# microsoft/XPretrain

Hardware: NVIDIA H100
Metric: video-text pairs/sec (12f x 224^2, 32 tok), CLIP-ViP ViT-B/16 fwd+InfoNCE+bwd (higher is better)
Workload: dtype bf16

## Files before the change

### xpretrain_b200/csrc/gemm.cu

```cuda
#include "../../include/xpretrain_b200.h"
#include "common.h"
#include "ptx.cuh"
#include <cstdlib>

namespace xp {

constexpr int BM = 128;
constexpr int BK = 64;
constexpr int MMA_K = 16;
constexpr int GEMM_THREADS = 384;

struct GemmDev {
  void* c;
  const float* bias;
  const __nv_bfloat16* residual;
  __nv_bfloat16* aux;
  int M, N, K;
  long long ldc, ldr, ld_aux;
  long long c_group, c_group_stride, r_group, r_group_stride;
  int act;
  int splits;
  int scale_cols;
  float alpha, col_scale;
  uint32_t mn_lbo, mn_sbo;
};

template <int BN>
struct GemmCfg {
  static constexpr int A_BYTES = BM * BK * 2;
  static constexpr int B_BYTES = BN * BK * 2;
  static constexpr int STAGE_BYTES = A_BYTES + B_BYTES;
  static constexpr int STAGES = (BN == 256) ? 4 : 6;
  static constexpr int SMEM_BYTES = STAGES * STAGE_BYTES + 1024 + 256;
};

__device__ __forceinline__ float act_gelu_erf(float x) { return 0.5f * x * (1.f + erff(x * 0.70710678118654752f)); }
__device__ __forceinline__ float act_gelu_erf_grad(float x) {
  float cdf = 0.5f * (1.f + erff(x * 0.70710678118654752f));
  float pdf = 0.3989422804014327f * __expf(-0.5f * x * x);
  return cdf + x * pdf;
}

template <int BN, int A_MN, int B_MN, int OUT, int ACT>
__global__ void __launch_bounds__(GEMM_THREADS, 1)
gemm_kernel(const __grid_constant__ CUtensorMap tmA, const __grid_constant__ CUtensorMap tmB, const GemmDev p) {
  using Cfg = GemmCfg<BN>;
  constexpr int STAGES = Cfg::STAGES;
  constexpr bool PINGPONG = BN == 128;
  constexpr int MH = PINGPONG ? 2 : 1;
  constexpr int NH = BN / 128;
  extern __shared__ uint8_t smem_raw[];
  const uint32_t raw_addr = smem_u32(smem_raw);
  uint8_t* smem = smem_raw + (((raw_addr + 1023u) & ~1023u) - raw_addr);
  uint64_t* full_bar = reinterpret_cast<uint64_t*>(smem + STAGES * Cfg::STAGE_BYTES);
  uint64_t* empty_bar = full_bar + STAGES;

  const int wg = threadIdx.x >> 7;
  const int lane = threadIdx.x & 31;

  const int num_m = (p.M + BM - 1) / BM;
  const int num_n = (p.N + BN - 1) / BN;
  const int num_mn = num_m * num_n;
  const int total = num_mn * p.splits;
  const int kb_total = (p.K + BK - 1) / BK;
  const int kb_per = (kb_total + p.splits - 1) / p.splits;

  if (threadIdx.x == 0) {
    tma_prefetch_desc(&tmA);
    tma_prefetch_desc(&tmB);
    for (int s = 0; s < STAGES; ++s) {
      mbar_init(&full_bar[s], 1);
      mbar_init(&empty_bar[s], PINGPONG ? 1 : 2);
    }
    fence_barrier_init();
  }
  __syncthreads();

  if (wg == 0) {
    setmaxnreg_dec<40>();
    if (threadIdx.x == 0) {
      int stage = 0;
      uint32_t phase = 0;
      for (int tile = blockIdx.x; tile < total; tile += gridDim.x) {
        const int split = tile / num_mn;
        const int mn = tile - split * num_mn;
        const int m_blk = mn / num_n;
        const int n_blk = mn - m_blk * num_n;
        const int k0 = split * kb_per;
        const int k1 = min(kb_total, k0 + kb_per);
        for (int kb = k0; kb < k1; ++kb) {
          mbar_wait_nocall(&empty_bar[stage], phase ^ 1);
          uint8_t* sA = smem + stage * Cfg::STAGE_BYTES;
          uint8_t* sB = sA + Cfg::A_BYTES;
          mbar_arrive_expect_tx(&full_bar[stage], Cfg::STAGE_BYTES);
          if (A_MN) {
#pragma unroll
            for (int i = 0; i < BM / 64; ++i)
              tma_load_2d(sA + i * (BK * 128), &tmA, &full_bar[stage], m_blk * BM + i * 64, kb * BK);
          } else {
            tma_load_2d(sA, &tmA, &full_bar[stage], kb * BK, m_blk * BM);
          }
          if (B_MN) {
#pragma unroll
            for (int i = 0; i < BN / 64; ++i)
              tma_load_2d(sB + i * (BK * 128), &tmB, &full_bar[stage], n_blk * BN + i * 64, kb * BK);
          } else {
            tma_load_2d(sB, &tmB, &full_bar[stage], kb * BK, n_blk * BN);
          }
          if (++stage == STAGES) {
            stage = 0;
            phase ^= 1;
          }
        }
      }
    }
  } else {
    setmaxnreg_inc<232>();
    const int cw = wg - 1;
    const int wq = (threadIdx.x >> 5) & 3;
    constexpr int act = ACT;
    const int N = p.N, scale_cols = p.scale_cols;
    const float alpha = p.alpha, col_scale = p.col_scale;
    __nv_bfloat16* const aux_p = p.aux;
    constexpr bool need_aux_in = (ACT == XP_ACT_DQUICK_GELU || ACT == XP_ACT_DGELU_ERF);
    const __nv_bfloat16* const xin_p = need_aux_in ? p.aux : p.residual;
    constexpr uint32_t A_OFF = 64 * 128;
    const int cta_tiles = (total - blockIdx.x + gridDim.x - 1) / gridDim.x;
    int stage = 0;
    uint32_t phase = 0;
    int local = 0;
    for (int tile = blockIdx.x; tile < total; tile += gridDim.x, ++local) {
      const int split = tile / num_mn;
      const int mn = tile - split * num_mn;
      const int m_blk = mn / num_n;
      const int n_blk = mn - m_blk * num_n;
      const int k0 = split * kb_per;
      const int k1 = min(kb_total, k0 + kb_per);
      if (PINGPONG && (local & 1) != cw) {
        const int next = stage + max(0, k1 - k0);
        phase ^= (next / STAGES) & 1;
        stage = next % STAGES;
        continue;
      }
      if (PINGPONG && local > 0) named_bar_sync(1 + cw, 256);
      const bool pass_turn = PINGPONG && local + 1 < cta_tiles;
      if (k0 >= k1) {
        if (pass_turn) named_bar_arrive(2 - cw, 256);
        continue;
      }
      float acc[MH * NH][64];
#pragma unroll
      for (int q = 0; q < MH * NH; ++q)
#pragma unroll
        for (int i = 0; i < 64; ++i) acc[q][i] = 0.f;
      int prev_stage = -1;
      for (int kb = k0; kb < k1; ++kb) {
        mbar_wait_nocall(&full_bar[stage], phase);
        const uint32_t sA = smem_u32(smem + stage * Cfg::STAGE_BYTES) + (PINGPONG ? 0 : cw * A_OFF);
        const uint32_t sB = smem_u32(smem + stage * Cfg::STAGE_BYTES) + Cfg::A_BYTES;
#pragma unroll
        for (int q = 0; q < MH * NH; ++q) wgmma_fence_regs(acc[q]);
        wgmma_fence();
#pragma unroll
        for (int j = 0; j < BK / MMA_K; ++j) {
#pragma unroll
          for (int mh = 0; mh < MH; ++mh) {
            const uint32_t am = sA + mh * A_OFF;
            const uint64_t adesc = A_MN ? make_smem_desc_sw128(am + j * (MMA_K * 128), p.mn_lbo, p.mn_sbo)
                                        : make_smem_desc_sw128(am + j * (MMA_K * 2), 16, 1024);
#pragma unroll
            for (int h = 0; h < NH; ++h) {
              const uint32_t bh = sB + h * (128 * 128);
              const uint64_t bdesc = B_MN ? make_smem_desc_sw128(bh + j * (MMA_K * 128), p.mn_lbo, p.mn_sbo)
                                          : make_smem_desc_sw128(bh + j * (MMA_K * 2), 16, 1024);
              wgmma_m64n128k16_bf16<A_MN, B_MN>(acc[mh * NH + h], adesc, bdesc);
            }
          }
        }
        wgmma_commit();
#pragma unroll
        for (int q = 0; q < MH * NH; ++q) wgmma_fence_regs(acc[q]);
        wgmma_wait<1>();
        if (prev_stage >= 0 && (threadIdx.x & 127) == 0) mbar_arrive(&empty_bar[prev_stage]);
        prev_stage = stage;
        if (++stage == STAGES) {
          stage = 0;
          phase ^= 1;
        }
      }
      if (pass_turn) named_bar_arrive(2 - cw, 256);
      const auto load_bias = [&](float2(&b)[16], int h) {
#pragma unroll
        for (int i = 0; i < 16; ++i) {
          const int n = n_blk * BN + h * 128 + i * 8 + (lane & 3) * 2;
          b[i] = make_float2(0.f, 0.f);
          if (p.bias != nullptr && split == 0 && n < N) b[i] = __ldg(reinterpret_cast<const float2*>(p.bias + n));
        }
      };
      constexpr bool bias_once = PINGPONG && !need_aux_in;
      float2 bias_tile[16];
      if (bias_once) load_bias(bias_tile, 0);
      wgmma_wait<0>();
#pragma unroll
      for (int q = 0; q < MH * NH; ++q) wgmma_fence_regs(acc[q]);
      if ((threadIdx.x & 127) == 0) mbar_arrive(&empty_bar[prev_stage]);

      const auto apply = [&](float& v0, float& v1, int n, uint32_t xg) -> uint32_t {
        if (n < scale_cols) {
          v0 *= col_scale;
          v1 *= col_scale;
        }
        uint32_t pre = 0;
        if (act == XP_ACT_QUICK_GELU) {
          pre = pack_bf16(v0, v1);
          v0 = quick_gelu(v0);
          v1 = quick_gelu(v1);
        } else if (act == XP_ACT_DQUICK_GELU) {
          v0 *= quick_gelu_grad(bf16_lo(xg));
          v1 *= quick_gelu_grad(bf16_hi(xg));
        } else if (act == XP_ACT_GELU_ERF) {
          pre = pack_bf16(v0, v1);
          v0 = act_gelu_erf(v0);
          v1 = act_gelu_erf(v1);
        } else if (act == XP_ACT_DGELU_ERF) {
          v0 *= act_gelu_erf_grad(bf16_lo(xg));
          v1 *= act_gelu_erf_grad(bf16_hi(xg));
        } else if (xin_p != nullptr) {
          v0 += bf16_lo(xg);
          v1 += bf16_hi(xg);
        }
        return pre;
      };
      constexpr bool save_pre = (ACT == XP_ACT_QUICK_GELU || ACT == XP_ACT_GELU_ERF);
      const int quad = lane & 3;
#pragma unroll
      for (int mh = 0; mh < MH; ++mh) {
        const int row_base = m_blk * BM + (PINGPONG ? mh : cw) * 64 + wq * 16 + (lane >> 2);
#pragma unroll
        for (int rr = 0; rr < 2; ++rr) {
          const int row = row_base + rr * 8;
          const bool row_ok = row < p.M;
          const long long c_off = p.c_group > 0 ? (row / p.c_group) * p.c_group_stride + (row % p.c_group) * p.ldc
                                                : static_cast<long long>(row) * p.ldc;
          const long long x_off = need_aux_in ? static_cast<long long>(row) * p.ld_aux
                                              : (p.r_group > 0 ? (row / p.r_group) * p.r_group_stride + (row % p.r_group) * p.ldr
                                                               : static_cast<long long>(row) * p.ldr);
          const long long a_off = static_cast<long long>(row) * p.ld_aux;
#pragma unroll
          for (int h = 0; h < NH; ++h) {
            const float* const a = acc[mh * NH + h];
            const int n_h = n_blk * BN + h * 128;
            float2 bias2[16];
            if (bias_once) {
#pragma unroll
              for (int i = 0; i < 16; ++i) bias2[i] = bias_tile[i];
            } else {
              load_bias(bias2, h);
            }
            if (OUT == XP_OUT_BF16) {
              uint32_t xin[4][4];
#pragma unroll
              for (int k = 0; k < 4; ++k) {
                const int n8 = n_h + (4 * k + quad) * 8;
                uint4 v = make_uint4(0u, 0u, 0u, 0u);
                if (xin_p != nullptr && row_ok && n8 < N) v = *reinterpret_cast<const uint4*>(xin_p + x_off + n8);
                xin[k][0] = v.x;
                xin[k][1] = v.y;
                xin[k][2] = v.z;
                xin[k][3] = v.w;
                if (xin_p != nullptr) quad_transpose(xin[k]);
              }
#pragma unroll
              for (int k = 0; k < 4; ++k) {
                uint32_t out[4], pre[4];
#pragma unroll
                for (int j = 0; j < 4; ++j) {
                  const int i = 4 * k + j;
                  float v0 = fmaf(a[4 * i + 2 * rr], alpha, bias2[i].x);
                  float v1 = fmaf(a[4 * i + 2 * rr + 1], alpha, bias2[i].y);
                  pre[j] = apply(v0, v1, n_h + i * 8 + quad * 2, xin[k][j]);
                  out[j] = pack_bf16(v0, v1);
                }
                const int n8 = n_h + (4 * k + quad) * 8;
                quad_transpose(out);
                if (row_ok && n8 < N)
                  *reinterpret_cast<uint4*>(static_cast<__nv_bfloat16*>(p.c) + c_off + n8) =
                      make_uint4(out[0], out[1], out[2], out[3]);
                if (save_pre && aux_p != nullptr) {
                  quad_transpose(pre);
                  if (row_ok && n8 < N)
                    *reinterpret_cast<uint4*>(aux_p + a_off + n8) = make_uint4(pre[0], pre[1], pre[2], pre[3]);
                }
              }
            } else if (row_ok) {
              uint32_t xin[16];
#pragma unroll
              for (int i = 0; i < 16; ++i) {
                const int n = n_h + i * 8 + quad * 2;
                xin[i] = 0;
                if (xin_p != nullptr && n < N) xin[i] = *reinterpret_cast<const uint32_t*>(xin_p + x_off + n);
              }
#pragma unroll
              for (int i = 0; i < 16; ++i) {
                const int n = n_h + i * 8 + quad * 2;
                if (n >= N) continue;
                float v0 = fmaf(a[4 * i + 2 * rr], alpha, bias2[i].x);
                float v1 = fmaf(a[4 * i + 2 * rr + 1], alpha, bias2[i].y);
                apply(v0, v1, n, xin[i]);
                if (OUT == XP_OUT_F32) {
                  *reinterpret_cast<float2*>(static_cast<float*>(p.c) + c_off + n) = make_float2(v0, v1);
                } else {
                  asm volatile("red.global.add.v2.f32 [%0], {%1, %2};" ::"l"(static_cast<float*>(p.c) + c_off + n),
                               "f"(v0), "f"(v1)
                               : "memory");
                }
              }
            }
          }
        }
      }
    }
  }
}

static int g_dbg_mn_lbo = 0, g_dbg_mn_sbo = 0;
}

extern "C" void xp_debug_gemm_mn_desc(int lbo, int sbo) {
  xp::g_dbg_mn_lbo = lbo;
  xp::g_dbg_mn_sbo = sbo;
}

extern "C" int xp_gemm(const XpGemm* g, void* stream_v) {
  using namespace xp;
  if (!g) return fail("xp_gemm: null args");
  cudaStream_t stream = static_cast<cudaStream_t>(stream_v);
  if (g->M <= 0 || g->N <= 0 || g->K <= 0) return fail("xp_gemm: M, N, K must be positive");
  if (g->N % 8 != 0) return fail("xp_gemm: N must be a multiple of 8");
  if (!g->a || !g->b || !g->c) return fail("xp_gemm: null operand");
  XP_ENTER(g->a);
  const int splits = g->splits <= 0 ? 1 : g->splits;
  if (splits > 1 && g->out != XP_OUT_F32_ATOMIC) return fail("xp_gemm: split-K requires XP_OUT_F32_ATOMIC");
  if ((g->act == XP_ACT_DQUICK_GELU || g->act == XP_ACT_DGELU_ERF) && !g->aux)
    return fail("xp_gemm: dGELU epilogue needs aux (the forward pre-activation)");
  if (g->act != XP_ACT_NONE && g->out != XP_OUT_BF16) return fail("xp_gemm: activation epilogues need a bf16 output");
  if (g->act != XP_ACT_NONE && g->residual)
    return fail("xp_gemm: a residual add cannot be combined with an activation epilogue");
  if (g->aux && g->c_group > 0) return fail("xp_gemm: aux cannot be combined with grouped rows (c_group > 0)");
  if (g->scale_cols < 0 || g->scale_cols % 2) return fail("xp_gemm: scale_cols must be even and non-negative");
  const int elem_c = g->out == XP_OUT_BF16 ? 2 : 4;
  if (!aligned(g->c, 16) || (g->ldc * elem_c) % 16)
    return fail("xp_gemm: C must be 16-byte aligned with a 16-byte multiple row pitch");
  if (g->bias && !aligned(g->bias, 16)) return fail("xp_gemm: bias must be 16-byte aligned");
  if (g->residual && (!aligned(g->residual, 16) || (g->ldr % 8)))
    return fail("xp_gemm: residual must be 16-byte aligned, ldr % 8 == 0");
  if (g->aux && (!aligned(g->aux, 16) || (g->ld_aux % 8)))
    return fail("xp_gemm: aux must be 16-byte aligned, ld_aux % 8 == 0");
  if ((g->c_group > 0 && g->c_group_stride % 8) || (g->r_group > 0 && g->r_group_stride % 8))
    return fail("xp_gemm: c_group_stride / r_group_stride must be multiples of 8 elements");

  const int nsm = sm_count();
  const int num_m = static_cast<int>((g->M + BM - 1) / BM);
  int bn = g->block_n;
  if (bn == 0) {
    const long long tiles256 = static_cast<long long>(num_m) * ((g->N + 255) / 256) * splits;
    const long long kb_split = ((g->K + BK - 1) / BK + splits - 1) / splits;
    const bool short_k_fwd = g->b_layout == 0 && kb_split <= 16;
    bn = (g->N >= 256 && tiles256 >= nsm && !short_k_fwd) ? 256 : 128;
  }
  const char* bad_bn = "xp_gemm: block_n must be 0, 128 or 256";
  if (bn != 128 && bn != 256) return fail(bad_bn);
  if (g->cta_pair < 0 || g->cta_pair > 1) return fail("xp_gemm: cta_pair must be 0 or 1 (no CTA pairs on sm_90)");
  const long long total = static_cast<long long>(num_m) * ((g->N + bn - 1) / bn) * splits;
  int grid = g->max_ctas > 0 ? g->max_ctas : nsm;
  if (grid < 1) grid = 1;
  if (grid > total) grid = static_cast<int>(total);

  CUtensorMap tmA, tmB;
  int rc;
  if (g->a_layout == 0)
    rc = make_tmap_bf16_2d(&tmA, g->a, g->K, g->M, g->lda, BK, BM);
  else
    rc = make_tmap_bf16_2d(&tmA, g->a, g->M, g->K, g->lda, 64, BK);
  if (rc) return rc;
  if (g->b_layout == 0)
    rc = make_tmap_bf16_2d(&tmB, g->b, g->K, g->N, g->ldb, BK, bn);
  else
    rc = make_tmap_bf16_2d(&tmB, g->b, g->N, g->K, g->ldb, 64, BK);
  if (rc) return rc;

  GemmDev dev;
  dev.c = g->c;
  dev.bias = g->bias;
  dev.residual = static_cast<const __nv_bfloat16*>(g->residual);
  dev.aux = static_cast<__nv_bfloat16*>(g->aux);
  dev.M = static_cast<int>(g->M);
  dev.N = static_cast<int>(g->N);
  dev.K = static_cast<int>(g->K);
  dev.ldc = g->ldc;
  dev.ldr = g->ldr;
  dev.ld_aux = g->ld_aux;
  dev.c_group = g->c_group;
  dev.c_group_stride = g->c_group_stride;
  dev.r_group = g->r_group;
  dev.r_group_stride = g->r_group_stride;
  dev.act = g->act;
  dev.splits = splits;
  dev.scale_cols = g->scale_cols;
  dev.alpha = g->alpha;
  dev.col_scale = g->col_scale;
  dev.mn_lbo = g_dbg_mn_lbo ? g_dbg_mn_lbo : BK * 128;
  dev.mn_sbo = g_dbg_mn_sbo ? g_dbg_mn_sbo : 1024;

  const char* bad_layout = "xp_gemm: a_layout/b_layout must be 0 or 1";
  auto launch = [&](auto tile_n, auto out, auto act) {
    return dispatch<0, 1>(g->a_layout, bad_layout, [&](auto a_mn) {
      return dispatch<0, 1>(g->b_layout, bad_layout, [&](auto b_mn) {
        constexpr auto kern = gemm_kernel<tile_n.value, a_mn.value, b_mn.value, out.value, act.value>;
        constexpr int smem = GemmCfg<tile_n.value>::SMEM_BYTES;
        if (smem_limit<kern>(smem)) return -1;
        kern<<<grid, GEMM_THREADS, smem, stream>>>(tmA, tmB, dev);
        XP_CHECK_LAUNCH("gemm_kernel");
        return 0;
      });
    });
  };
  using no_act = std::integral_constant<int, XP_ACT_NONE>;
  return dispatch<256, 128>(bn, bad_bn, [&](auto tile_n) {
    return dispatch<XP_OUT_BF16, XP_OUT_F32, XP_OUT_F32_ATOMIC>(g->out, "xp_gemm: bad out mode", [&](auto out) {
      if constexpr (out.value != XP_OUT_BF16)
        return launch(tile_n, out, no_act{});
      else
        return dispatch<XP_ACT_NONE, XP_ACT_QUICK_GELU, XP_ACT_DQUICK_GELU, XP_ACT_GELU_ERF, XP_ACT_DGELU_ERF>(
            g->act, "xp_gemm: bad act", [&](auto act) { return launch(tile_n, out, act); });
    });
  });
}
```

### xpretrain_b200/csrc/ptx.cuh

```cuda
#pragma once
#include <cuda.h>
#include <cuda_bf16.h>
#include <cuda_fp16.h>
#include <cuda_runtime.h>
#include <stdint.h>
#include <stdio.h>

namespace xp {

#ifndef XP_WAIT_TIMEOUT_CYCLES
#define XP_WAIT_TIMEOUT_CYCLES (8000000000ll)
#endif

__device__ __forceinline__ uint32_t smem_u32(const void* p) {
  return static_cast<uint32_t>(__cvta_generic_to_shared(p));
}
__device__ __forceinline__ int lane_id() { return threadIdx.x & 31; }

__device__ __forceinline__ void mbar_init(uint64_t* bar, uint32_t count) {
  asm volatile("mbarrier.init.shared::cta.b64 [%0], %1;" ::"r"(smem_u32(bar)), "r"(count) : "memory");
}
__device__ __forceinline__ void fence_barrier_init() {
  asm volatile("fence.mbarrier_init.release.cluster;" ::: "memory");
}
__device__ __forceinline__ void fence_proxy_async_smem() {
  asm volatile("fence.proxy.async.shared::cta;" ::: "memory");
}
__device__ __forceinline__ void mbar_arrive_expect_tx(uint64_t* bar, uint32_t bytes) {
  asm volatile("mbarrier.arrive.expect_tx.shared::cta.b64 _, [%0], %1;" ::"r"(smem_u32(bar)), "r"(bytes)
               : "memory");
}
__device__ __forceinline__ void mbar_arrive(uint64_t* bar) {
  asm volatile("mbarrier.arrive.shared::cta.b64 _, [%0];" ::"r"(smem_u32(bar)) : "memory");
}
__device__ __forceinline__ bool mbar_try_wait(uint64_t* bar, uint32_t parity) {
  uint32_t ok;
  asm volatile(
      "{\n"
      ".reg .pred p;\n"
      "mbarrier.try_wait.parity.shared::cta.b64 p, [%1], %2;\n"
      "selp.u32 %0, 1, 0, p;\n"
      "}\n"
      : "=r"(ok)
      : "r"(smem_u32(bar)), "r"(parity)
      : "memory");
  return ok != 0;
}
__device__ __forceinline__ void mbar_wait(uint64_t* bar, uint32_t parity) {
  if (mbar_try_wait(bar, parity)) return;
  long long t0 = clock64();
  while (!mbar_try_wait(bar, parity)) {
    if (clock64() - t0 > XP_WAIT_TIMEOUT_CYCLES) {
      printf("xpretrain_b200: mbarrier wait timeout (block %d thread %d parity %u)\n", blockIdx.x, threadIdx.x,
             parity);
      __trap();
    }
  }
}
__device__ __forceinline__ void mbar_wait_nocall(uint64_t* bar, uint32_t parity) {
  if (mbar_try_wait(bar, parity)) return;
  long long t0 = clock64();
  while (!mbar_try_wait(bar, parity)) {
    if (clock64() - t0 > XP_WAIT_TIMEOUT_CYCLES) __trap();
  }
}

__device__ __forceinline__ void tma_prefetch_desc(const CUtensorMap* m) {
  asm volatile("prefetch.tensormap [%0];" ::"l"(reinterpret_cast<uint64_t>(m)) : "memory");
}
__device__ __forceinline__ void tma_load_2d(void* smem_dst, const CUtensorMap* m, uint64_t* bar, int c0, int c1) {
  asm volatile(
      "cp.async.bulk.tensor.2d.shared::cluster.global.mbarrier::complete_tx::bytes [%0], [%1, {%3, %4}], [%2];"
      ::"r"(smem_u32(smem_dst)), "l"(reinterpret_cast<uint64_t>(m)), "r"(smem_u32(bar)), "r"(c0), "r"(c1)
      : "memory");
}
__device__ __forceinline__ void tma_load_3d(void* smem_dst, const CUtensorMap* m, uint64_t* bar, int c0, int c1,
                                            int c2) {
  asm volatile(
      "cp.async.bulk.tensor.3d.shared::cluster.global.mbarrier::complete_tx::bytes [%0], [%1, {%3, %4, %5}], [%2];"
      ::"r"(smem_u32(smem_dst)), "l"(reinterpret_cast<uint64_t>(m)), "r"(smem_u32(bar)), "r"(c0), "r"(c1), "r"(c2)
      : "memory");
}

__device__ __forceinline__ void tma_store_2d(const CUtensorMap* m, uint32_t smem_src, int c0, int c1) {
  asm volatile("cp.async.bulk.tensor.2d.global.shared::cta.bulk_group [%0, {%2, %3}], [%1];" ::"l"(
                   reinterpret_cast<uint64_t>(m)),
               "r"(smem_src), "r"(c0), "r"(c1)
               : "memory");
}
__device__ __forceinline__ void tma_store_commit() { asm volatile("cp.async.bulk.commit_group;" ::: "memory"); }
template <int N>
__device__ __forceinline__ void tma_store_wait_read() {
  asm volatile("cp.async.bulk.wait_group.read %0;" ::"n"(N) : "memory");
}

__device__ __forceinline__ void wgmma_fence() { asm volatile("wgmma.fence.sync.aligned;" ::: "memory"); }
__device__ __forceinline__ void wgmma_commit() { asm volatile("wgmma.commit_group.sync.aligned;" ::: "memory"); }
template <int N>
__device__ __forceinline__ void wgmma_wait() {
  asm volatile("wgmma.wait_group.sync.aligned %0;" ::"n"(N) : "memory");
}
template <int R>
__device__ __forceinline__ void wgmma_fence_regs(float (&d)[R]) {
#pragma unroll
  for (int i = 0; i < R; ++i) asm volatile("" : "+f"(d[i])::"memory");
}

template <int TA, int TB>
__device__ __forceinline__ void wgmma_m64n128k16_bf16(float (&d)[64], uint64_t adesc, uint64_t bdesc) {
  asm volatile(
      "wgmma.mma_async.sync.aligned.m64n128k16.f32.bf16.bf16 {"
      "%0, %1, %2, %3, %4, %5, %6, %7, %8, %9, %10, %11, %12, %13, %14, %15, "
      "%16, %17, %18, %19, %20, %21, %22, %23, %24, %25, %26, %27, %28, %29, %30, %31, "
      "%32, %33, %34, %35, %36, %37, %38, %39, %40, %41, %42, %43, %44, %45, %46, %47, "
      "%48, %49, %50, %51, %52, %53, %54, %55, %56, %57, %58, %59, %60, %61, %62, %63"
      "}, %64, %65, 1, 1, 1, %66, %67;"
      : "+f"(d[0]), "+f"(d[1]), "+f"(d[2]), "+f"(d[3]), "+f"(d[4]), "+f"(d[5]), "+f"(d[6]), "+f"(d[7]),
        "+f"(d[8]), "+f"(d[9]), "+f"(d[10]), "+f"(d[11]), "+f"(d[12]), "+f"(d[13]), "+f"(d[14]), "+f"(d[15]),
        "+f"(d[16]), "+f"(d[17]), "+f"(d[18]), "+f"(d[19]), "+f"(d[20]), "+f"(d[21]), "+f"(d[22]), "+f"(d[23]),
        "+f"(d[24]), "+f"(d[25]), "+f"(d[26]), "+f"(d[27]), "+f"(d[28]), "+f"(d[29]), "+f"(d[30]), "+f"(d[31]),
        "+f"(d[32]), "+f"(d[33]), "+f"(d[34]), "+f"(d[35]), "+f"(d[36]), "+f"(d[37]), "+f"(d[38]), "+f"(d[39]),
        "+f"(d[40]), "+f"(d[41]), "+f"(d[42]), "+f"(d[43]), "+f"(d[44]), "+f"(d[45]), "+f"(d[46]), "+f"(d[47]),
        "+f"(d[48]), "+f"(d[49]), "+f"(d[50]), "+f"(d[51]), "+f"(d[52]), "+f"(d[53]), "+f"(d[54]), "+f"(d[55]),
        "+f"(d[56]), "+f"(d[57]), "+f"(d[58]), "+f"(d[59]), "+f"(d[60]), "+f"(d[61]), "+f"(d[62]), "+f"(d[63])
      : "l"(adesc), "l"(bdesc), "n"(TA), "n"(TB));
}

template <int TA, int TB>
__device__ __forceinline__ void wgmma_m64n64k16_ss(float (&d)[32], uint64_t adesc, uint64_t bdesc) {
  asm volatile(
      "wgmma.mma_async.sync.aligned.m64n64k16.f32.bf16.bf16 {"
      "%0, %1, %2, %3, %4, %5, %6, %7, %8, %9, %10, %11, %12, %13, %14, %15, "
      "%16, %17, %18, %19, %20, %21, %22, %23, %24, %25, %26, %27, %28, %29, %30, %31"
      "}, %32, %33, 1, 1, 1, %34, %35;"
      : "+f"(d[0]), "+f"(d[1]), "+f"(d[2]), "+f"(d[3]), "+f"(d[4]), "+f"(d[5]), "+f"(d[6]), "+f"(d[7]),
        "+f"(d[8]), "+f"(d[9]), "+f"(d[10]), "+f"(d[11]), "+f"(d[12]), "+f"(d[13]), "+f"(d[14]), "+f"(d[15]),
        "+f"(d[16]), "+f"(d[17]), "+f"(d[18]), "+f"(d[19]), "+f"(d[20]), "+f"(d[21]), "+f"(d[22]), "+f"(d[23]),
        "+f"(d[24]), "+f"(d[25]), "+f"(d[26]), "+f"(d[27]), "+f"(d[28]), "+f"(d[29]), "+f"(d[30]), "+f"(d[31])
      : "l"(adesc), "l"(bdesc), "n"(TA), "n"(TB));
}
template <int TB>
__device__ __forceinline__ void wgmma_m64n64k16_rs(float (&d)[32], const uint32_t (&a)[4], uint64_t bdesc) {
  asm volatile(
      "wgmma.mma_async.sync.aligned.m64n64k16.f32.bf16.bf16 {"
      "%0, %1, %2, %3, %4, %5, %6, %7, %8, %9, %10, %11, %12, %13, %14, %15, "
      "%16, %17, %18, %19, %20, %21, %22, %23, %24, %25, %26, %27, %28, %29, %30, %31"
      "}, {%32, %33, %34, %35}, %36, 1, 1, 1, %37;"
      : "+f"(d[0]), "+f"(d[1]), "+f"(d[2]), "+f"(d[3]), "+f"(d[4]), "+f"(d[5]), "+f"(d[6]), "+f"(d[7]),
        "+f"(d[8]), "+f"(d[9]), "+f"(d[10]), "+f"(d[11]), "+f"(d[12]), "+f"(d[13]), "+f"(d[14]), "+f"(d[15]),
        "+f"(d[16]), "+f"(d[17]), "+f"(d[18]), "+f"(d[19]), "+f"(d[20]), "+f"(d[21]), "+f"(d[22]), "+f"(d[23]),
        "+f"(d[24]), "+f"(d[25]), "+f"(d[26]), "+f"(d[27]), "+f"(d[28]), "+f"(d[29]), "+f"(d[30]), "+f"(d[31])
      : "r"(a[0]), "r"(a[1]), "r"(a[2]), "r"(a[3]), "l"(bdesc), "n"(TB));
}

template <uint32_t N>
__device__ __forceinline__ void setmaxnreg_dec() {
  asm volatile("setmaxnreg.dec.sync.aligned.u32 %0;" ::"n"(N));
}
template <uint32_t N>
__device__ __forceinline__ void setmaxnreg_inc() {
  asm volatile("setmaxnreg.inc.sync.aligned.u32 %0;" ::"n"(N));
}
__device__ __forceinline__ void named_bar_sync(uint32_t id, uint32_t threads) {
  asm volatile("bar.sync %0, %1;" ::"r"(id), "r"(threads) : "memory");
}
__device__ __forceinline__ void named_bar_arrive(uint32_t id, uint32_t threads) {
  asm volatile("bar.arrive %0, %1;" ::"r"(id), "r"(threads) : "memory");
}

__device__ __forceinline__ uint64_t make_smem_desc_sw128(uint32_t smem_addr, uint32_t lbo_bytes,
                                                         uint32_t sbo_bytes) {
  uint64_t d = 0;
  d |= static_cast<uint64_t>((smem_addr & 0x3FFFF) >> 4);
  d |= static_cast<uint64_t>((lbo_bytes >> 4) & 0x3FFF) << 16;
  d |= static_cast<uint64_t>((sbo_bytes >> 4) & 0x3FFF) << 32;
  d |= static_cast<uint64_t>(1) << 62;
  return d;
}

__device__ __forceinline__ void quad_transpose(uint32_t (&v)[4]) {
  const int q = threadIdx.x & 3;
  uint32_t out[4];
  out[0] = out[1] = out[2] = out[3] = 0u;
#pragma unroll
  for (int t = 0; t < 4; ++t) {
    const int j = q ^ t;
    const uint32_t send = j == 0 ? v[0] : j == 1 ? v[1] : j == 2 ? v[2] : v[3];
    const uint32_t got = t == 0 ? send : __shfl_xor_sync(0xffffffffu, send, t);
#pragma unroll
    for (int c = 0; c < 4; ++c)
      if (c == j) out[c] = got;
  }
#pragma unroll
  for (int c = 0; c < 4; ++c) v[c] = out[c];
}

__device__ __forceinline__ uint32_t pack_bf16(float lo, float hi) {
  __nv_bfloat162 v = __floats2bfloat162_rn(lo, hi);
  return *reinterpret_cast<uint32_t*>(&v);
}
__device__ __forceinline__ float bf16_lo(uint32_t v) { return __uint_as_float(v << 16); }
__device__ __forceinline__ float bf16_hi(uint32_t v) { return __uint_as_float(v & 0xFFFF0000u); }

__device__ __forceinline__ void unpack8_bf16(const uint4& u, float (&f)[8]) {
  f[0] = bf16_lo(u.x); f[1] = bf16_hi(u.x); f[2] = bf16_lo(u.y); f[3] = bf16_hi(u.y);
  f[4] = bf16_lo(u.z); f[5] = bf16_hi(u.z); f[6] = bf16_lo(u.w); f[7] = bf16_hi(u.w);
}
__device__ __forceinline__ uint4 pack8_bf16(const float (&f)[8]) {
  uint4 u;
  u.x = pack_bf16(f[0], f[1]); u.y = pack_bf16(f[2], f[3]); u.z = pack_bf16(f[4], f[5]); u.w = pack_bf16(f[6], f[7]);
  return u;
}
__device__ __forceinline__ void unpack8_f16(const uint4& u, float (&f)[8]) {
  const __half2* h = reinterpret_cast<const __half2*>(&u);
#pragma unroll
  for (int i = 0; i < 4; ++i) {
    const float2 v = __half22float2(h[i]);
    f[2 * i] = v.x;
    f[2 * i + 1] = v.y;
  }
}
__device__ __forceinline__ uint4 pack8_f16_satfinite(const float (&f)[8]) {
  uint4 u;
  uint32_t* w = reinterpret_cast<uint32_t*>(&u);
#pragma unroll
  for (int i = 0; i < 4; ++i)
    asm("cvt.rn.satfinite.f16x2.f32 %0, %1, %2;" : "=r"(w[i]) : "f"(f[2 * i + 1]), "f"(f[2 * i]));
  return u;
}
__device__ __forceinline__ void load8(const float* p, float (&f)[8]) {
  const float4 a = *reinterpret_cast<const float4*>(p), b = *reinterpret_cast<const float4*>(p + 4);
  f[0] = a.x; f[1] = a.y; f[2] = a.z; f[3] = a.w; f[4] = b.x; f[5] = b.y; f[6] = b.z; f[7] = b.w;
}
__device__ __forceinline__ void load8(const __nv_bfloat16* p, float (&f)[8]) {
  unpack8_bf16(*reinterpret_cast<const uint4*>(p), f);
}
__device__ __forceinline__ void load8(const __half* p, float (&f)[8]) {
  const uint4 u = *reinterpret_cast<const uint4*>(p);
  unpack8_f16(u, f);
}
__device__ __forceinline__ void store8(float* p, const float (&f)[8]) {
  *reinterpret_cast<float4*>(p) = make_float4(f[0], f[1], f[2], f[3]);
  *reinterpret_cast<float4*>(p + 4) = make_float4(f[4], f[5], f[6], f[7]);
}
__device__ __forceinline__ void store8(__nv_bfloat16* p, const float (&f)[8]) {
  *reinterpret_cast<uint4*>(p) = pack8_bf16(f);
}
__device__ __forceinline__ void store8_satfinite(__half* p, const float (&f)[8]) {
  *reinterpret_cast<uint4*>(p) = pack8_f16_satfinite(f);
}

template <typename T>
__device__ __forceinline__ float to_f32(T v) { return static_cast<float>(v); }
template <>
__device__ __forceinline__ float to_f32<__nv_bfloat16>(__nv_bfloat16 v) { return __bfloat162float(v); }
template <>
__device__ __forceinline__ float to_f32<__half>(__half v) { return __half2float(v); }
template <typename T>
__device__ __forceinline__ T from_f32(float v);
template <>
__device__ __forceinline__ float from_f32<float>(float v) { return v; }
template <>
__device__ __forceinline__ __nv_bfloat16 from_f32<__nv_bfloat16>(float v) { return __float2bfloat16(v); }
template <>
__device__ __forceinline__ __half from_f32<__half>(float v) { return __float2half(v); }

template <typename T>
__device__ __forceinline__ T warp_sum(T v) {
#pragma unroll
  for (int o = 16; o > 0; o >>= 1) v += __shfl_xor_sync(0xffffffffu, v, o);
  return v;
}
__device__ __forceinline__ float warp_max(float v) {
#pragma unroll
  for (int o = 16; o > 0; o >>= 1) v = fmaxf(v, __shfl_xor_sync(0xffffffffu, v, o));
  return v;
}

__device__ __forceinline__ float fast_sigmoid(float y) {
  float t;
  asm("tanh.approx.f32 %0, %1;" : "=f"(t) : "f"(0.5f * y));
  return fmaf(0.5f, t, 0.5f);
}
__device__ __forceinline__ float quick_gelu(float x) { return x * fast_sigmoid(1.702f * x); }
__device__ __forceinline__ float quick_gelu_grad(float x) {
  float y = 1.702f * x;
  y = y > 64.f ? 64.f : (y < -64.f ? -64.f : y);
  const float s = fast_sigmoid(y);
  return s * fmaf(y, 1.f - s, 1.f);
}

}
```

Baseline: 290.3.

## Stage GEMM epilogue aux tensors through shared memory with TMA loads and stores

For the QuickGELU-backward GEMM with 128-wide tiles, the producer warp now TMA-prefetches the saved pre-activation tile into two double-buffered shared-memory slots, guarded by new mbarriers, so the consumer epilogue reads it from swizzled smem instead of uncoalesced global loads. The forward QuickGELU GEMM can write both its output and pre-activation tiles through smem via TMA bulk stores. Both paths give up one pipeline stage to make room for the slots, and the DQuickGELU case is no longer allowed to pick 256-wide tiles. Compile-time probe switches that skip epilogue loads and stores are also added, defaulting to off.

```diff
diff --git a/xpretrain_b200/csrc/gemm.cu b/xpretrain_b200/csrc/gemm.cu
--- a/xpretrain_b200/csrc/gemm.cu
+++ b/xpretrain_b200/csrc/gemm.cu
@@ -2,6 +2,10 @@
 #include "common.h"
 #include "ptx.cuh"
 #include <cstdlib>
+
+#ifndef XP_GEMM_PROBE
+#define XP_GEMM_PROBE 0
+#endif
 
 namespace xp {
 
@@ -25,14 +29,24 @@
   uint32_t mn_lbo, mn_sbo;
 };
 
-template <int BN>
+__host__ __device__ constexpr bool pre_in_smem(int bn, int act) { return bn == 128 && act == XP_ACT_DQUICK_GELU; }
+
+template <int BN, bool EPI_SMEM = false>
 struct GemmCfg {
   static constexpr int A_BYTES = BM * BK * 2;
   static constexpr int B_BYTES = BN * BK * 2;
   static constexpr int STAGE_BYTES = A_BYTES + B_BYTES;
-  static constexpr int STAGES = (BN == 256) ? 4 : 6;
-  static constexpr int SMEM_BYTES = STAGES * STAGE_BYTES + 1024 + 256;
+  static constexpr int PRE_BYTES = BM * 128 * 2;
+  static constexpr int PRE_SLOTS = EPI_SMEM ? 2 : 0;
+  static constexpr int STAGES = (BN == 256) ? 4 : (EPI_SMEM ? 5 : 6);
+  static constexpr int PRE_OFF = STAGES * STAGE_BYTES;
+  static constexpr int BAR_BYTES = 256;
+  static constexpr int SMEM_BYTES = PRE_OFF + PRE_SLOTS * PRE_BYTES + 1024 + BAR_BYTES;
+  static_assert(PRE_OFF % 1024 == 0, "pre-activation slots must stay 1 KiB aligned");
+  static_assert((2 * STAGES + 2 * PRE_SLOTS) * 8 <= BAR_BYTES, "mbarriers do not fit");
+  static_assert(SMEM_BYTES <= 227 * 1024, "past the 227 KiB per-block shared-memory opt-in limit of sm_90");
 };
+static_assert(GemmCfg<128, true>::SMEM_BYTES == 230656, "shared-memory budget changed: update the comment above");
 
 __device__ __forceinline__ float act_gelu_erf(float x) { return 0.5f * x * (1.f + erff(x * 0.70710678118654752f)); }
 __device__ __forceinline__ float act_gelu_erf_grad(float x) {
@@ -41,10 +55,13 @@
   return cdf + x * pdf;
 }
 
-template <int BN, int A_MN, int B_MN, int OUT, int ACT>
+template <int BN, int A_MN, int B_MN, int OUT, int ACT, bool TMA_OUT = false>
 __global__ void __launch_bounds__(GEMM_THREADS, 1)
-gemm_kernel(const __grid_constant__ CUtensorMap tmA, const __grid_constant__ CUtensorMap tmB, const GemmDev p) {
-  using Cfg = GemmCfg<BN>;
+gemm_kernel(const __grid_constant__ CUtensorMap tmA, const __grid_constant__ CUtensorMap tmB,
+            const __grid_constant__ CUtensorMap tmX, const __grid_constant__ CUtensorMap tmC, const GemmDev p) {
+  constexpr bool PRE_SMEM = pre_in_smem(BN, ACT);
+  static_assert(!TMA_OUT || (BN == 128 && OUT == XP_OUT_BF16 && ACT == XP_ACT_QUICK_GELU), "TMA_OUT: QuickGELU only");
+  using Cfg = GemmCfg<BN, PRE_SMEM || TMA_OUT>;
   constexpr int STAGES = Cfg::STAGES;
   constexpr bool PINGPONG = BN == 128;
   constexpr int MH = PINGPONG ? 2 : 1;
@@ -52,8 +69,10 @@
   extern __shared__ uint8_t smem_raw[];
   const uint32_t raw_addr = smem_u32(smem_raw);
   uint8_t* smem = smem_raw + (((raw_addr + 1023u) & ~1023u) - raw_addr);
-  uint64_t* full_bar = reinterpret_cast<uint64_t*>(smem + STAGES * Cfg::STAGE_BYTES);
+  uint64_t* full_bar = reinterpret_cast<uint64_t*>(smem + Cfg::PRE_OFF + Cfg::PRE_SLOTS * Cfg::PRE_BYTES);
   uint64_t* empty_bar = full_bar + STAGES;
+  uint64_t* pre_full = empty_bar + STAGES;
+  uint64_t* pre_empty = pre_full + 2;
 
   const int wg = threadIdx.x >> 7;
   const int lane = threadIdx.x & 31;
@@ -72,6 +91,13 @@
       mbar_init(&full_bar[s], 1);
       mbar_init(&empty_bar[s], PINGPONG ? 1 : 2);
     }
+    if (PRE_SMEM) {
+      tma_prefetch_desc(&tmX);
+      for (int s = 0; s < Cfg::PRE_SLOTS; ++s) {
+        mbar_init(&pre_full[s], 1);
+        mbar_init(&pre_empty[s], 128);
+      }
+    }
     fence_barrier_init();
   }
   __syncthreads();
@@ -81,14 +107,27 @@
     if (threadIdx.x == 0) {
       int stage = 0;
       uint32_t phase = 0;
-      for (int tile = blockIdx.x; tile < total; tile += gridDim.x) {
+      int local = 0;
+      for (int tile = blockIdx.x; tile < total; tile += gridDim.x, ++local) {
         const int split = tile / num_mn;
         const int mn = tile - split * num_mn;
         const int m_blk = mn / num_n;
         const int n_blk = mn - m_blk * num_n;
         const int k0 = split * kb_per;
         const int k1 = min(kb_total, k0 + kb_per);
+        const int pre_slot = local & 1;
+        const uint32_t pre_parity = ((local >> 1) & 1) ^ 1;
+        bool pre_issued = !PRE_SMEM;
+        const auto issue_pre = [&]() {
+          uint8_t* sX = smem + Cfg::PRE_OFF + pre_slot * Cfg::PRE_BYTES;
+          mbar_arrive_expect_tx(&pre_full[pre_slot], Cfg::PRE_BYTES);
+#pragma unroll
+          for (int i = 0; i < 2; ++i)
+            tma_load_2d(sX + i * (BM * 128), &tmX, &pre_full[pre_slot], n_blk * BN + i * 64, m_blk * BM);
+          pre_issued = true;
+        };
         for (int kb = k0; kb < k1; ++kb) {
+          if (!pre_issued && mbar_test_wait(&pre_empty[pre_slot], pre_parity)) issue_pre();
           mbar_wait_nocall(&empty_bar[stage], phase ^ 1);
           uint8_t* sA = smem + stage * Cfg::STAGE_BYTES;
           uint8_t* sB = sA + Cfg::A_BYTES;
@@ -111,6 +150,10 @@
             stage = 0;
             phase ^= 1;
           }
+        }
+        if (!pre_issued) {
+          mbar_wait_nocall(&pre_empty[pre_slot], pre_parity);
+          issue_pre();
         }
       }
     }
@@ -197,13 +240,15 @@
           if (p.bias != nullptr && split == 0 && n < N) b[i] = __ldg(reinterpret_cast<const float2*>(p.bias + n));
         }
       };
-      constexpr bool bias_once = PINGPONG && !need_aux_in;
+      constexpr bool bias_once = PINGPONG && !need_aux_in && !TMA_OUT;
       float2 bias_tile[16];
       if (bias_once) load_bias(bias_tile, 0);
       wgmma_wait<0>();
 #pragma unroll
       for (int q = 0; q < MH * NH; ++q) wgmma_fence_regs(acc[q]);
       if ((threadIdx.x & 127) == 0) mbar_arrive(&empty_bar[prev_stage]);
+      const uint8_t* const sX = smem + Cfg::PRE_OFF + cw * Cfg::PRE_BYTES;
+      if (PRE_SMEM) mbar_wait_nocall(&pre_full[cw], (local >> 1) & 1);
 
       const auto apply = [&](float& v0, float& v1, int n, uint32_t xg) -> uint32_t {
         if (n < scale_cols) {
@@ -233,6 +278,44 @@
       };
       constexpr bool save_pre = (ACT == XP_ACT_QUICK_GELU || ACT == XP_ACT_GELU_ERF);
       const int quad = lane & 3;
+      if (TMA_OUT) {
+        uint8_t* const sO = smem + Cfg::PRE_OFF + cw * Cfg::PRE_BYTES;
+        const bool leader = (threadIdx.x & 127) == 0;
+#pragma unroll
+        for (int mh = 0; mh < MH; ++mh) {
+          if (leader) tma_store_wait_read<0>();
+          named_bar_sync(3 + cw, 128);
+          const float* const a = acc[mh];
+#pragma unroll
+          for (int i = 0; i < 16; ++i) {
+            const int n = n_blk * BN + i * 8 + quad * 2;
+            float2 b = make_float2(0.f, 0.f);
+            if (p.bias != nullptr && n < N) b = __ldg(reinterpret_cast<const float2*>(p.bias + n));
+#pragma unroll
+            for (int rr = 0; rr < 2; ++rr) {
+              const int rl = wq * 16 + (lane >> 2) + rr * 8;
+              float v0 = fmaf(a[4 * i + 2 * rr], alpha, b.x);
+              float v1 = fmaf(a[4 * i + 2 * rr + 1], alpha, b.y);
+              const uint32_t pre = apply(v0, v1, n, 0u);
+              const int off = (i >> 3) * (64 * 128) + rl * 128 + (((i & 7) ^ (rl & 7)) << 4) + quad * 4;
+              *reinterpret_cast<uint32_t*>(sO + off) = pack_bf16(v0, v1);
+              *reinterpret_cast<uint32_t*>(sO + 2 * (64 * 128) + off) = pre;
+            }
+          }
+          fence_proxy_async_smem();
+          named_bar_sync(3 + cw, 128);
+          if (leader) {
+            const int row0 = m_blk * BM + mh * 64, col0 = n_blk * BN;
+#pragma unroll
+            for (int b = 0; b < 2; ++b) {
+              tma_store_2d(&tmC, smem_u32(sO + b * (64 * 128)), col0 + b * 64, row0);
+              tma_store_2d(&tmX, smem_u32(sO + (2 + b) * (64 * 128)), col0 + b * 64, row0);
+            }
+            tma_store_commit();
+          }
+        }
+        continue;
+      }
 #pragma unroll
       for (int mh = 0; mh < MH; ++mh) {
         const int row_base = m_blk * BM + (PINGPONG ? mh : cw) * 64 + wq * 16 + (lane >> 2);
@@ -259,16 +342,33 @@
             }
             if (OUT == XP_OUT_BF16) {
               uint32_t xin[4][4];
-#pragma unroll
-              for (int k = 0; k < 4; ++k) {
-                const int n8 = n_h + (4 * k + quad) * 8;
-                uint4 v = make_uint4(0u, 0u, 0u, 0u);
-                if (xin_p != nullptr && row_ok && n8 < N) v = *reinterpret_cast<const uint4*>(xin_p + x_off + n8);
-                xin[k][0] = v.x;
-                xin[k][1] = v.y;
-                xin[k][2] = v.z;
-                xin[k][3] = v.w;
-                if (xin_p != nullptr) quad_transpose(xin[k]);
+              if (PRE_SMEM) {
+                const int rl = mh * 64 + wq * 16 + (lane >> 2) + rr * 8;
+#pragma unroll
+                for (int k = 0; k < 4; ++k)
+#pragma unroll
+                  for (int j = 0; j < 4; ++j) {
+                    const int i = 4 * k + j;
+                    xin[k][j] = *reinterpret_cast<const uint32_t*>(sX + (i >> 3) * (BM * 128) + rl * 128 +
+                                                                   (((i & 7) ^ (rl & 7)) << 4) + quad * 4);
+                  }
+              } else {
+#pragma unroll
+                for (int k = 0; k < 4; ++k) {
+                  const int n8 = n_h + (4 * k + quad) * 8;
+                  uint4 v = make_uint4(0u, 0u, 0u, 0u);
+                  if (XP_GEMM_PROBE == 3 && need_aux_in) {
+                    const uint32_t c = pack_bf16(col_scale, col_scale);
+                    v = make_uint4(c, c, c, c);
+                  } else if (xin_p != nullptr && row_ok && n8 < N) {
+                    v = *reinterpret_cast<const uint4*>(xin_p + x_off + n8);
+                  }
+                  xin[k][0] = v.x;
+                  xin[k][1] = v.y;
+                  xin[k][2] = v.z;
+                  xin[k][3] = v.w;
+                  if (xin_p != nullptr) quad_transpose(xin[k]);
+                }
               }
 #pragma unroll
               for (int k = 0; k < 4; ++k) {
@@ -283,10 +383,10 @@
                 }
                 const int n8 = n_h + (4 * k + quad) * 8;
                 quad_transpose(out);
-                if (row_ok && n8 < N)
+                if (row_ok && n8 < N && !(XP_GEMM_PROBE == 2 && save_pre))
                   *reinterpret_cast<uint4*>(static_cast<__nv_bfloat16*>(p.c) + c_off + n8) =
                       make_uint4(out[0], out[1], out[2], out[3]);
-                if (save_pre && aux_p != nullptr) {
+                if (save_pre && aux_p != nullptr && XP_GEMM_PROBE != 1) {
                   quad_transpose(pre);
                   if (row_ok && n8 < N)
                     *reinterpret_cast<uint4*>(aux_p + a_off + n8) = make_uint4(pre[0], pre[1], pre[2], pre[3]);
@@ -319,7 +419,9 @@
           }
         }
       }
+      if (PRE_SMEM) mbar_arrive(&pre_empty[cw]);
     }
+    if (TMA_OUT && (threadIdx.x & 127) == 0) tma_store_wait_all();
   }
 }
 
@@ -366,7 +468,7 @@
     const long long tiles256 = static_cast<long long>(num_m) * ((g->N + 255) / 256) * splits;
     const long long kb_split = ((g->K + BK - 1) / BK + splits - 1) / splits;
     const bool short_k_fwd = g->b_layout == 0 && kb_split <= 16;
-    bn = (g->N >= 256 && tiles256 >= nsm && !short_k_fwd) ? 256 : 128;
+    bn = (g->N >= 256 && tiles256 >= nsm && !short_k_fwd && g->act != XP_ACT_DQUICK_GELU) ? 256 : 128;
   }
   const char* bad_bn = "xp_gemm: block_n must be 0, 128 or 256";
   if (bn != 128 && bn != 256) return fail(bad_bn);
@@ -388,6 +490,12 @@
   else
     rc = make_tmap_bf16_2d(&tmB, g->b, g->N, g->K, g->ldb, 64, BK);
   if (rc) return rc;
+  const bool tma_out = bn == 128 && g->act == XP_ACT_QUICK_GELU && g->out == XP_OUT_BF16 && g->aux && g->c_group == 0;
+  CUtensorMap tmX = {}, tmC = {};
+  if (pre_in_smem(bn, g->act) && (rc = make_tmap_bf16_2d(&tmX, g->aux, g->N, g->M, g->ld_aux, 64, BM))) return rc;
+  if (tma_out && ((rc = make_tmap_bf16_2d(&tmX, g->aux, g->N, g->M, g->ld_aux, 64, 64)) ||
+                  (rc = make_tmap_bf16_2d(&tmC, g->c, g->N, g->M, g->ldc, 64, 64))))
+    return rc;
 
   GemmDev dev;
   dev.c = g->c;
@@ -413,17 +521,24 @@
   dev.mn_sbo = g_dbg_mn_sbo ? g_dbg_mn_sbo : 1024;
 
   const char* bad_layout = "xp_gemm: a_layout/b_layout must be 0 or 1";
-  auto launch = [&](auto tile_n, auto out, auto act) {
+  auto launch_as = [&](auto tile_n, auto out, auto act, auto staged) {
     return dispatch<0, 1>(g->a_layout, bad_layout, [&](auto a_mn) {
       return dispatch<0, 1>(g->b_layout, bad_layout, [&](auto b_mn) {
-        constexpr auto kern = gemm_kernel<tile_n.value, a_mn.value, b_mn.value, out.value, act.value>;
-        constexpr int smem = GemmCfg<tile_n.value>::SMEM_BYTES;
+        constexpr auto kern = gemm_kernel<tile_n.value, a_mn.value, b_mn.value, out.value, act.value, staged.value>;
+        constexpr bool epi_smem = pre_in_smem(tile_n.value, act.value) || staged.value;
+        constexpr int smem = GemmCfg<tile_n.value, epi_smem>::SMEM_BYTES;
         if (smem_limit<kern>(smem)) return -1;
-        kern<<<grid, GEMM_THREADS, smem, stream>>>(tmA, tmB, dev);
+        kern<<<grid, GEMM_THREADS, smem, stream>>>(tmA, tmB, tmX, tmC, dev);
         XP_CHECK_LAUNCH("gemm_kernel");
         return 0;
       });
     });
+  };
+  auto launch = [&](auto tile_n, auto out, auto act) {
+    if constexpr (tile_n.value == 128 && out.value == XP_OUT_BF16 && act.value == XP_ACT_QUICK_GELU) {
+      if (tma_out) return launch_as(tile_n, out, act, std::true_type{});
+    }
+    return launch_as(tile_n, out, act, std::false_type{});
   };
   using no_act = std::integral_constant<int, XP_ACT_NONE>;
   return dispatch<256, 128>(bn, bad_bn, [&](auto tile_n) {
diff --git a/xpretrain_b200/csrc/ptx.cuh b/xpretrain_b200/csrc/ptx.cuh
--- a/xpretrain_b200/csrc/ptx.cuh
+++ b/xpretrain_b200/csrc/ptx.cuh
@@ -39,6 +39,19 @@
       "{\n"
       ".reg .pred p;\n"
       "mbarrier.try_wait.parity.shared::cta.b64 p, [%1], %2;\n"
+      "selp.u32 %0, 1, 0, p;\n"
+      "}\n"
+      : "=r"(ok)
+      : "r"(smem_u32(bar)), "r"(parity)
+      : "memory");
+  return ok != 0;
+}
+__device__ __forceinline__ bool mbar_test_wait(uint64_t* bar, uint32_t parity) {
+  uint32_t ok;
+  asm volatile(
+      "{\n"
+      ".reg .pred p;\n"
+      "mbarrier.test_wait.parity.shared::cta.b64 p, [%1], %2;\n"
       "selp.u32 %0, 1, 0, p;\n"
       "}\n"
       : "=r"(ok)
@@ -93,6 +106,7 @@
 __device__ __forceinline__ void tma_store_wait_read() {
   asm volatile("cp.async.bulk.wait_group.read %0;" ::"n"(N) : "memory");
 }
+__device__ __forceinline__ void tma_store_wait_all() { asm volatile("cp.async.bulk.wait_group 0;" ::: "memory"); }
 
 __device__ __forceinline__ void wgmma_fence() { asm volatile("wgmma.fence.sync.aligned;" ::: "memory"); }
 __device__ __forceinline__ void wgmma_commit() { asm volatile("wgmma.commit_group.sync.aligned;" ::: "memory"); }
```

Measured after the change: 301.1, median of 6. +3.7%, better.
